# NVlabs/long-video-gan

Measured on NVIDIA H100. Metric: frames/sec (G+D train step: every convolution and torch_utils.ops call of the forward/backward passes, replayed), higher is better.
Workload: dtype f32

## Files before the change

### long-video-gan_b200/csrc/conv_igemm.cu

```cuda

#include <algorithm>
#include <cuda.h>
#include <stdlib.h>

#include "common.cuh"
#include "wgmma.cuh"
#include "conv_engine.cuh"

namespace lvg {
bool pw_supported(int dtype, int groups, int cin, int cout, int kt, int kh, int kw, int pad_t, int pad_h, int pad_w, int stride, int64_t P);
int pw_conv(const float* x, const float* w, float* y, int n, int cin, int cout, int64_t P, int64_t w_sco, int64_t w_sci, cudaStream_t s);
bool pw_tc_supported(int dtype, int groups, int cin, int cout, int kt, int kh, int kw, int pad_t, int pad_h, int pad_w, int stride, int64_t P);
int pw_tc_conv(const void* x, const void* w, void* y, int dtype, int n, int ck, int cm, int64_t P, int64_t w_sm, int64_t w_sk, void* workspace,
               int64_t workspace_bytes, cudaStream_t s, const void* res = nullptr, float rscale = 1.f);
int64_t pw_tc_workspace(int dtype, int ck, int cm);
}

namespace lvg {
namespace {

using namespace tc;

constexpr int kBM = 128;
constexpr int kATile = kBM * 16 * 2;
// ... 679 lines not shown
        set_error("convnd_fprop: outside the tensor-core kernel's envelope");
        return LVG_UNSUPPORTED;
    }
    IgemmJob j = fprop_job(sh, x, w, y);
    j.bias = bias; j.act = act; j.alpha = alpha; j.gain = gain; j.clamp = clamp;
    return run_igemm(j, workspace, workspace_bytes, (cudaStream_t)stream);
}

extern "C" int lvg_convnd_dgrad(const void* dy, const void* w, void* dx, int dtype, int n, int groups, int cin, int cout, int t, int h, int wd,
                                int kt, int kh, int kw, int pad_t, int pad_h, int pad_w, int stride, void* workspace, int64_t workspace_bytes,
                                void* stream)
{
    LVG_REQUIRE(dy && w && dx, "convnd_dgrad: dy, w, dx must not be NULL");
    const int route = lvg_convnd_route(1, dtype, n, groups, cin, cout, t, h, wd, kt, kh, kw, pad_t, pad_h, pad_w, stride, 0);
    if (route == 1) return pw_conv((const float*)dy, (const float*)w, (float*)dx, n, cout, cin, (int64_t)t * h * wd, 1, cin, (cudaStream_t)stream);
    if (route == 2 && aligned16(dy) && aligned16(dx))
        return pw_tc_conv(dy, w, dx, dtype, n, cout, cin, (int64_t)t * h * wd, 1, cin, workspace, workspace_bytes, (cudaStream_t)stream);
    const ConvShape sh = {dtype, n, groups, cin, cout, t, h, wd, kt, kh, kw, pad_t, pad_h, pad_w, stride};
    if (!sh.dgrad_ok()) {
        set_error("convnd_dgrad: outside the tensor-core kernel's envelope");
        return LVG_UNSUPPORTED;
    }
    return run_igemm(dgrad_job(sh, dy, w, dx), workspace, workspace_bytes, (cudaStream_t)stream);
}



namespace lvg {
namespace {

struct WgradV2Params {
    void* dw;
    int out_f32;
    int bf16, split;
    int n, groups, cin, cout;
    int to, ho;
    int kt, kh, kw, pad_t, pad_h, pad_w;
    int nt;
    int nblk_a, nblk_b;
    int lo_a, lo_b;
    int nseg, seg_w[4], seg_x0[4], ps[4];
    int rh;
    int khc;
    int ablk;
    int nsplit;
    int a_bytes, b_bytes, stage_bytes, stages;
    int64_t split_stride;
    int mrows;
    int tail_bytes;
};

struct WgradMaps { CUtensorMap a[4]; CUtensorMap b; };

template <bool BF16, int TAPS, int NT>
__global__ void __launch_bounds__(kIgemmThreads, 1) conv_wgrad_v2_kernel(const __grid_constant__ WgradMaps maps, const WgradV2Params p)
{
    extern __shared__ __align__(128) unsigned char smem_raw[];
    __shared__ uint64_t full_bar[kMaxStages], empty_bar[kMaxStages];
    unsigned char* smem = reinterpret_cast<unsigned char*>((reinterpret_cast<uintptr_t>(smem_raw) + 127) & ~(uintptr_t)127);

    const int warp = threadIdx.x / 32, lane = threadIdx.x % 32;
    const int wg = __shfl_sync(0xffffffffu, (int)threadIdx.x / 128, 0);
    int bx = blockIdx.x;
    const int sp = bx % p.nsplit; bx /= p.nsplit;
    int ky0 = 0;
    if (p.khc == 1) { ky0 = bx % p.kh; bx /= p.kh; }
    const int kt = bx % p.kt;
    const int nti = bx / p.kt;
    const int mti = blockIdx.y, g = blockIdx.z;
    const int nop = p.split ? 2 : 1;
    const int consumers = p.mrows / 64;

    const int rblocks = (p.ho + p.rh - 1) / p.rh;
    const int per_plane = p.nseg * rblocks;
    const int total = p.n * p.to * per_plane;
    const int s0 = (int)((int64_t)total * sp / p.nsplit), s1 = (int)((int64_t)total * (sp + 1) / p.nsplit);

    if (threadIdx.x == 0) {
        for (int s = 0; s < p.stages; s++) { mbar_init(&full_bar[s], 1); mbar_init(&empty_bar[s], (uint32_t)consumers); }
        fence_barrier_init();
    }
    for (int i = threadIdx.x; i < (p.stages * p.stage_bytes + p.tail_bytes) / 16; i += kIgemmThreads) reinterpret_cast<uint4*>(smem)[i] = make_uint4(0u, 0u, 0u, 0u);
    fence_proxy_async();
    __syncthreads();

    if (wg == 0) {
        if (warp == 0 && elect_one()) {
            for (int s = s0; s < s1; s++) {
                const int it = s - s0, slot = it % p.stages;
                if (it >= p.stages) mbar_wait(&empty_bar[slot], (uint32_t)((it / p.stages - 1) & 1));
                int r = s;
                const int rb = r % rblocks; r /= rblocks;
                const int seg = r % p.nseg; r /= p.nseg;
                const int t = r % p.to;
                const int n = r / p.to;
                const int inst = n * p.groups + g;
                unsigned char* st = smem + (size_t)slot * p.stage_bytes;
                mbar_expect_tx(&full_bar[slot], (uint32_t)(nop * (p.a_bytes + p.b_bytes)));
                const int oy0 = rb * p.rh;
                for (int o = 0; o < nop; o++) {
                    tma_load_4d(st + (size_t)o * p.a_bytes, &maps.a[seg], 0, oy0, t, inst * p.nblk_a + o * p.lo_a + mti * 16, &full_bar[slot]);
                    tma_load_4d(st + (size_t)nop * p.a_bytes + (size_t)o * p.b_bytes, &maps.b, 2 * (p.seg_x0[seg] - p.pad_w), oy0 + ky0 - p.pad_h,
                                t + kt - p.pad_t, inst * p.nblk_b + o * p.lo_b + nti * (NT / 8), &full_bar[slot]);
                }
            }
        }
    } else if (wg >= 1 && wg - 1 < consumers) {
        const int cw = wg - 1;
        const int tid = threadIdx.x % 128, wq = tid / 32;
        float acc[TAPS][NT / 2];
#pragma unroll
        for (int tap = 0; tap < TAPS; tap++)
#pragma unroll
            for (int i = 0; i < NT / 2; i++) acc[tap][i] = 0.f;
        int prev = -1;
        for (int s = s0; s < s1; s++) {
            const int it = s - s0, slot = it % p.stages;
            const int seg = (s / rblocks) % p.nseg;
            const int rb = s % rblocks;
            const int rows = min(p.rh, p.ho - rb * p.rh);
            const int ksteps = (rows * p.ps[seg] + 15) / 16;
            const uint32_t blk_a = (uint32_t)(p.rh * p.ps[seg] * 16);
            const uint32_t blk_b = (uint32_t)((p.rh + p.khc - 1) * p.ps[seg] * 16);
            const uint32_t ky16 = (uint32_t)p.ps[seg];
            mbar_wait(&full_bar[slot], (uint32_t)((it / p.stages) & 1));
            wgmma_fence();
            const uint32_t a0 = smem_u32(smem + (size_t)slot * p.stage_bytes) + (uint32_t)cw * 8u * blk_a;
            const uint32_t b0 = smem_u32(smem + (size_t)slot * p.stage_bytes) + (uint32_t)(nop * p.a_bytes);
            const uint32_t a_hi = desc_hi(blk_a), b_hi = desc_hi(blk_b);
            for (int term = 0; term < (p.split ? 3 : 1); term++) {
                const uint32_t a_lo0 = desc_lo(a0 + (term == 1 ? (uint32_t)p.a_bytes : 0u), 128);
                const uint32_t b_lo0 = desc_lo(b0 + (term == 2 ? (uint32_t)p.b_bytes : 0u), 128);
                for (int k = 0; k < ksteps; k++) {
#pragma unroll
                    for (int tap = 0; tap < TAPS; tap++) {
                        const int kyi = tap / p.kw, kx = tap - kyi * p.kw;
                        wgmma_m64nNk16<BF16, NT, 1, 1>(acc[tap], a_lo0 + 16u * k, a_hi, b_lo0 + 16u * k + (uint32_t)kyi * ky16 + (uint32_t)kx, b_hi);
                    }
                }
            }
            wgmma_commit();
            wgmma_wait<1>();
            mbar_arrive_if(&empty_bar[prev >= 0 ? prev : 0], prev >= 0 && tid == 0);
            prev = slot;
        }
        wgmma_wait<0>();

        const int taps = p.kt * p.kh * p.kw;
        const int ci0 = nti * NT;
#pragma unroll
        for (int tap = 0; tap < TAPS; tap++) {
            const int kyi = tap / p.kw, kx = tap - kyi * p.kw;
            const int tapg = (kt * p.kh + ky0 + kyi) * p.kw + kx;
#pragma unroll
            for (int i = 0; i < NT / 2; i++) {
                const int co = mti * kBM + cw * 64 + wq * 16 + lane / 4 + 8 * ((i / 2) % 2);
                const int cil = (i / 4) * 8 + 2 * (lane % 4) + i % 2;
                if (co >= p.cout || ci0 + cil >= p.cin) continue;
                const int64_t off = (((int64_t)g * p.cout + co) * p.cin + ci0 + cil) * taps + tapg;
                const float v = acc[tap][i];
                if (p.nsplit > 1) reinterpret_cast<float*>(p.dw)[(int64_t)sp * p.split_stride + off] = v;
                else if (p.out_f32) reinterpret_cast<float*>(p.dw)[off] = v;
                else reinterpret_cast<__half*>(p.dw)[off] = __float2half_rn(v);
            }
        }
    }
}

template <class TOut>
__global__ void __launch_bounds__(256) conv_wgrad_reduce_kernel(const float* __restrict__ part, TOut* __restrict__ out, int64_t n, int nsplit, int64_t stride)
{
    for (int64_t i = (int64_t)blockIdx.x * blockDim.x + threadIdx.x; i < n; i += (int64_t)gridDim.x * blockDim.x) {
        float s = 0.f;
        for (int k = 0; k < nsplit; k++) s += part[(int64_t)k * stride + i];
        if constexpr (sizeof(TOut) == 2) out[i] = __float2half_rn(s);
        else out[i] = s;
    }
}

inline int wgrad_cpad_a(int cout) { return (cout < kBM && env_flag("LVG_WGRAD_COMPACT", 1)) ? round_up(cout, 16) : round_up(cout, kBM); }

}

WgradPlan wgrad_plan(const ConvShape& s, bool fold)
{
    const int cin = s.cin, cout = s.cout, kh = s.kh, kw = s.kw;
    const int to = s.to(), ho = s.ho(), wo = s.wo();
    WgradPlan q;
    q.split = s.split();
    q.cpad_a = wgrad_cpad_a(cout);
    q.ablk = q.cpad_a < kBM ? q.cpad_a / 8 : 16;
    q.mrows = (q.cpad_a <= 64 && env_flag("LVG_WGRAD_M64", 1)) ? 64 : kBM;
    q.cpad_b = round_up(cin, 16);
    q.khc = (fold && kh > 1 && kh * kw * 32 <= 256 && cin <= env_flag("LVG_WGRAD_FOLD_CIN", 32) && env_flag("LVG_WGRAD_FOLD", 1)) ? kh : 1;
    int nt_cap = (256 / (q.khc * kw)) / 32 * 32;
// ... 12 lines not shown
        const int min_rows = q.ps % 16 != 0 ? 2 : 1;
        while (nt_cap > 32 && 2 * stage_of(min_rows, nt_cap) > 200 * 1024) nt_cap -= 32;
    }
    q.ntiles = (q.cpad_b + nt_cap - 1) / nt_cap;
    q.nt = round_up((q.cpad_b + q.ntiles - 1) / q.ntiles, 32);
    q.cpad_b = q.nt * q.ntiles;
    q.mt = (q.cpad_a + kBM - 1) / kBM;
    const int64_t inst = s.inst();
    q.a_bytes = inst * nop * (q.cpad_a / 8) * (int64_t)to * ho * wo * 16;
    q.b_bytes = inst * nop * (q.cpad_b / 8) * s.thw() * 16;
    q.dw_elems = (int64_t)s.groups * cout * cin * s.taps();
    q.rh = 1;
    while (q.rh < ho && q.rh < 255 - q.khc && stage_of(q.rh + 1, q.nt) <= 80 * 1024) q.rh++;
    if (q.ps % 16 != 0) q.rh = q.rh >= 2 ? q.rh / 2 * 2 : 2;
    for (;;) {
        q.a_stage = q.ablk * q.rh * q.ps * 16;
        q.b_stage = (q.nt / 8) * (q.rh + q.khc - 1) * q.ps * 16;
        q.stage_bytes = round_up(nop * (q.a_stage + q.b_stage), 128);
        const int over = (nop - 1) * q.a_stage + (q.mrows / 8) * q.rh * q.ps * 16 - q.stage_bytes;
        q.tail_bytes = round_up(256 + (over > 0 ? over : 0), 128);
        const int step = q.ps % 16 != 0 ? 2 : 1;
        if (2 * q.stage_bytes + q.tail_bytes <= 220 * 1024 || q.rh <= step) break;
        q.rh -= step;
    }
    q.stages = 2;
    while (q.stages < kMaxStages && (q.stages + 1) * q.stage_bytes + q.tail_bytes <= 220 * 1024) q.stages++;
    q.smem = (size_t)q.stages * q.stage_bytes + q.tail_bytes + 128;
    if (q.khc > 1 && q.smem > 227 * 1024) return wgrad_plan(s, false);
    const int64_t ctas = (int64_t)q.ntiles * (kh / q.khc) * s.kt * q.mt * s.groups;
    const int64_t stages = (int64_t)s.n * to * q.nseg * ((ho + q.rh - 1) / q.rh);
    const int sms = num_sms();
    int64_t cap = 160;
    if (cap > stages) cap = stages;
    while (cap > 1 && cap * q.dw_elems * 4 > (256ll << 20)) cap--;
    int64_t ns = 1;
    double best = 1e300;
    for (int64_t k = 1; k <= cap; k++) {
        const int64_t waves = (ctas * k + sms - 1) / sms;
        const double tm = (double)waves * ((double)((stages + k - 1) / k) + 4.0 * q.khc);
        if (tm < best * 0.999) { best = tm; ns = k; }
    }
    {
        const char* e = getenv("LVG_WGRAD_NSPLIT");
        if (e && atoi(e) >= 1) ns = atoi(e) < stages ? atoi(e) : stages;
    }
    q.nsplit = (int)ns;
    q.part_bytes = q.nsplit > 1 ? q.nsplit * q.dw_elems * 4 : 0;
    return q;
}

namespace {

typedef void (*WgradKernel)(const WgradMaps, const WgradV2Params);
template <bool B>
WgradKernel wgrad_kernel_of(int taps, int nt)
{
    switch (taps * 1000 + nt) {
    case 1032: return conv_wgrad_v2_kernel<B, 1, 32>;
    case 1064: return conv_wgrad_v2_kernel<B, 1, 64>;
    case 1096: return conv_wgrad_v2_kernel<B, 1, 96>;
    case 1128: return conv_wgrad_v2_kernel<B, 1, 128>;
    case 2032: return conv_wgrad_v2_kernel<B, 2, 32>;
    case 2064: return conv_wgrad_v2_kernel<B, 2, 64>;
    case 2096: return conv_wgrad_v2_kernel<B, 2, 96>;
    case 2128: return conv_wgrad_v2_kernel<B, 2, 128>;
    case 3032: return conv_wgrad_v2_kernel<B, 3, 32>;
    case 3064: return conv_wgrad_v2_kernel<B, 3, 64>;
    case 4032: return conv_wgrad_v2_kernel<B, 4, 32>;
    case 4064: return conv_wgrad_v2_kernel<B, 4, 64>;
    case 5032: return conv_wgrad_v2_kernel<B, 5, 32>;
    case 6032: return conv_wgrad_v2_kernel<B, 6, 32>;
    case 7032: return conv_wgrad_v2_kernel<B, 7, 32>;
    case 8032: return conv_wgrad_v2_kernel<B, 8, 32>;
    }
    if constexpr (!B) {
        switch (taps * 1000 + nt) {
        case 1160: return conv_wgrad_v2_kernel<B, 1, 160>;
        case 1192: return conv_wgrad_v2_kernel<B, 1, 192>;
        case 1224: return conv_wgrad_v2_kernel<B, 1, 224>;
        case 1256: return conv_wgrad_v2_kernel<B, 1, 256>;
        }
    }
    return nullptr;
}
WgradKernel wgrad_kernel(int split, int taps, int nt) { return split ? wgrad_kernel_of<true>(taps, nt) : wgrad_kernel_of<false>(taps, nt); }

bool dy8_tiles_agree(const ConvShape& s) { return wgrad_cpad_a(s.cout) == round_up(s.cout, 16); }

}

WgradRooms wgrad_rooms(const WgradPlan& q, bool dy8_pre) { return {dy8_pre ? 0 : round256(q.a_bytes), round256(q.b_bytes), q.part_bytes}; }

int run_wgrad(const ConvShape& sh, const void* x, const void* dy, void* dw, const WgradInputs& in, void* workspace, int64_t workspace_bytes,
              cudaStream_t s)
{
    const int to = sh.to(), ho = sh.ho(), wo = sh.wo();
    const WgradPlan q = wgrad_plan(sh);
    const WgradRooms r = wgrad_rooms(q, in.dy8_pre != nullptr);
    LVG_REQUIRE(workspace && workspace_bytes >= r.total(), "convnd_wgrad: workspace too small");
    LVG_REQUIRE(aligned16(workspace), "convnd_wgrad: workspace must be 16-byte aligned");
    LVG_REQUIRE(sh.groups <= 65535 && q.mt <= 65535, "convnd_wgrad: too many groups / channel tiles");
    const int64_t inst = sh.inst();
    unsigned char* ws = reinterpret_cast<unsigned char*>(workspace);
    unsigned char* dy8 = in.dy8_pre ? const_cast<unsigned char*>(in.dy8_pre) : ws;
    unsigned char* x8 = in.x8_pre ? const_cast<unsigned char*>(in.x8_pre) : ws + r.dy8;
    float* part = reinterpret_cast<float*>(ws + r.dy8 + r.x8);
    const int64_t thw_a = (int64_t)to * ho * wo, thw_b = sh.thw();
    {
        int rc = in.dy8_pre ? LVG_OK : pack_act(dy, dy8, q.split, inst, sh.cout, q.cpad_a / 8, to, sh.hos(), sh.wos(), ho, wo, sh.stride, s, in.dy_scale);
        if (rc) return rc;
        rc = in.x8_pre ? LVG_OK : pack_act(x, x8, q.split, inst, sh.cin, q.cpad_b / 8, sh.t, sh.h, sh.wd, sh.h, sh.wd, 1, s, in.x_scale);
        if (rc) return rc;
    }
    WgradV2Params p;
    memset(&p, 0, sizeof(p));
    p.out_f32 = q.split; p.bf16 = q.split; p.split = q.split;
    p.n = sh.n; p.groups = sh.groups; p.cin = sh.cin; p.cout = sh.cout; p.to = to; p.ho = ho;
    p.kt = sh.kt; p.kh = sh.kh; p.kw = sh.kw; p.pad_t = sh.pad_t; p.pad_h = sh.pad_h; p.pad_w = sh.pad_w;
    p.nt = q.nt;
    p.nblk_a = (q.split ? 2 : 1) * (q.cpad_a / 8); p.nblk_b = (q.split ? 2 : 1) * (q.cpad_b / 8);
    p.lo_a = q.cpad_a / 8; p.lo_b = q.cpad_b / 8;
    p.nseg = q.nseg;
    for (int j = 0; j < 4; j++) { p.seg_w[j] = q.seg_w[j]; p.seg_x0[j] = q.seg_x0[j]; p.ps[j] = q.ps; }
    p.rh = q.rh; p.khc = q.khc; p.ablk = q.ablk;
    p.mrows = q.mrows;
    p.a_bytes = q.a_stage; p.b_bytes = q.b_stage; p.stage_bytes = q.stage_bytes; p.stages = q.stages; p.tail_bytes = q.tail_bytes;
    const size_t smem = q.smem;
    LVG_REQUIRE(smem <= 227 * 1024, "convnd_wgrad: stage does not fit shared memory (%zu bytes)", smem);
    p.nsplit = q.nsplit;
    p.split_stride = q.dw_elems;
    p.dw = q.nsplit > 1 ? (void*)part : dw;
    WgradMaps maps;
    memset(&maps, 0, sizeof(maps));
    for (int j = 0; j < p.nseg; j++) {
        const int rc = encode_map(&maps.a[j], dy8 + (size_t)p.seg_x0[j] * 16, p.seg_w[j], ho, to, inst * p.nblk_a, wo, (int64_t)ho * wo, thw_a,
                                  p.ps[j], p.rh, 1, q.ablk);
        if (rc) return rc;
    }
    {
        const int rc = encode_map(&maps.b, x8, sh.wd, sh.h, sh.t, inst * p.nblk_b, sh.wd, (int64_t)sh.h * sh.wd, thw_b, p.ps[0], p.rh + q.khc - 1, 1,
                                  q.nt / 8);
        if (rc) return rc;
    }
    void (*const kern)(const WgradMaps, const WgradV2Params) = wgrad_kernel(q.split, q.khc * sh.kw, q.nt);
    LVG_REQUIRE(kern != nullptr, "convnd_wgrad: no kernel for %d taps x %d columns (split %d)", q.khc * sh.kw, q.nt, q.split);
    LVG_CUDA(cudaFuncSetAttribute(kern, cudaFuncAttributeMaxDynamicSharedMemorySize, (int)smem));
    dim3 grid((unsigned)(q.ntiles * sh.kt * (sh.kh / q.khc) * q.nsplit), (unsigned)q.mt, (unsigned)sh.groups);
    kern<<<grid, kIgemmThreads, smem, s>>>(maps, p);
    LVG_LAUNCH_CHECK();
    if (q.nsplit > 1) {
        int64_t blocks = (q.dw_elems + 255) / 256;
        const int64_t cap = (int64_t)num_sms() * 32;
        if (blocks > cap) blocks = cap;
        if (q.split) conv_wgrad_reduce_kernel<float><<<(unsigned)blocks, 256, 0, s>>>(part, (float*)dw, q.dw_elems, q.nsplit, q.dw_elems);
        else conv_wgrad_reduce_kernel<__half><<<(unsigned)blocks, 256, 0, s>>>(part, (__half*)dw, q.dw_elems, q.nsplit, q.dw_elems);
        LVG_LAUNCH_CHECK();
    }
    return LVG_OK;
}

bool shares_dy8(const ConvShape& s) { return env_flag("LVG_CONV_SHARED_DY8", 1) && dy8_tiles_agree(s); }

BackwardRooms backward_rooms(const ConvShape& s, bool shared)
{
    const Geometry gd = job_geometry(dgrad_job(s, nullptr, nullptr, nullptr));
    const WgradRooms wr = wgrad_rooms(wgrad_plan(s), shared);
    return {shared ? round256(gd.act_bytes) : 0, std::max(igemm_rooms_of(gd, shared).total(), wr.total()), wr.dy8};
}

int64_t backward_workspace(const ConvShape& s)
{
    const int64_t sep = backward_rooms(s, false).total();
    return dy8_tiles_agree(s) ? std::max(sep, backward_rooms(s, true).total()) : sep;
}

int backward_dgrad(const ConvShape& s, const void* dy, const float* d, const void* w, void* dx, void* workspace, int64_t workspace_bytes,
                   cudaStream_t st, Backward& b)
{
    const bool shared = shares_dy8(s);
    const BackwardRooms r = backward_rooms(s, shared);
    LVG_REQUIRE(workspace && aligned16(workspace) && workspace_bytes >= r.total(), "convnd backward: workspace too small or misaligned");
    unsigned char* ws = reinterpret_cast<unsigned char*>(workspace);
    b.dy8 = shared ? ws : nullptr;
    b.rest = ws + r.dy8;
    b.rest_bytes = workspace_bytes - r.dy8;
    b.x8 = b.rest + r.x8;
    IgemmJob j = dgrad_job(s, dy, w, dx);
    if (shared) {
        const int rc = pack_act(dy, ws, s.split(), s.inst(), s.cout, job_geometry(j).cblk, s.to(), s.hos(), s.wos(), s.ho(), s.wo(), s.stride, st, d);
        if (rc) return rc;
        j.x8_pre = ws;
    } else {
        j.in_scale = d;
    }
    return run_igemm(j, b.rest, b.rest_bytes, st);
}

int backward_wgrad(const ConvShape& s, const Backward& b, const void* x, const void* dy, const float* d, void* dw, const float* x_scale,
// ... 112 lines not shown
```

### long-video-gan_b200/csrc/wgmma.cuh

```cuda
#pragma once
#include "common.cuh"

namespace lvg {
namespace tc {

__device__ __forceinline__ uint32_t smem_u32(const void* p) { return (uint32_t)__cvta_generic_to_shared(p); }

__device__ __forceinline__ bool elect_one()
{
    uint32_t pred = 0;
    asm volatile(
        "{\n"
        " .reg .pred p;\n"
        " elect.sync _|p, 0xffffffff;\n"
        " selp.u32 %0, 1, 0, p;\n"
        "}\n"
        : "=r"(pred));
    return pred != 0;
}

__device__ __forceinline__ void mbar_init(uint64_t* bar, uint32_t count)
{
    asm volatile("mbarrier.init.shared::cta.b64 [%0], %1;" ::"r"(smem_u32(bar)), "r"(count));
}
// ... 25 lines not shown
__device__ __forceinline__ void bulk_copy_g2s(void* dst_smem, const void* src_gmem, uint32_t bytes, uint64_t* bar)
{
    asm volatile("cp.async.bulk.shared::cluster.global.mbarrier::complete_tx::bytes [%0], [%1], %2, [%3];" ::"r"(smem_u32(dst_smem)),
                 "l"(src_gmem), "r"(bytes), "r"(smem_u32(bar))
                 : "memory");
}
__device__ __forceinline__ void fence_barrier_init() { asm volatile("fence.mbarrier_init.release.cluster;" ::: "memory"); }
__device__ __forceinline__ void fence_proxy_async() { asm volatile("fence.proxy.async.shared::cta;" ::: "memory"); }

__device__ __forceinline__ uint32_t desc_lo(uint32_t saddr, uint32_t lbo_bytes) { return ((saddr >> 4) & 0x3fffu) | (((lbo_bytes >> 4) & 0x3fffu) << 16); }
__device__ __forceinline__ uint32_t desc_hi(uint32_t sbo_bytes) { return (sbo_bytes >> 4) & 0x3fffu; }

__device__ __forceinline__ void wgmma_fence() { asm volatile("wgmma.fence.sync.aligned;" ::: "memory"); }
__device__ __forceinline__ void wgmma_commit() { asm volatile("wgmma.commit_group.sync.aligned;" ::: "memory"); }
template <int N>
__device__ __forceinline__ void wgmma_wait() { asm volatile("wgmma.wait_group.sync.aligned %0;" ::"n"(N) : "memory"); }

#define LVG_D8(i)                                                                                                            \
    "+f"(d[i]), "+f"(d[i + 1]), "+f"(d[i + 2]), "+f"(d[i + 3]), "+f"(d[i + 4]), "+f"(d[i + 5]), "+f"(d[i + 6]), "+f"(d[i + 7])
#define LVG_WGMMA_ASM(NS, TYPE, REGS, A0, A1, B0, B1, TA_, TB_, SC)                                                           \
    "{\n .reg .b64 da, db;\n .reg .pred p;\n setp.ne.b32 p, %" SC ", 0;\n mov.b64 da, {%" A0 ", %" A1 "};\n"                   \
    " mov.b64 db, {%" B0 ", %" B1 "};\n wgmma.mma_async.sync.aligned.m64n" NS "k16.f32." TYPE "." TYPE " " REGS                 \
    ", da, db, p, 1, 1, %" TA_ ", %" TB_ ";\n}\n"
#define LVG_WGMMA(NS, REGS, A0, A1, B0, B1, TA_, TB_, SC, ...)                                                                \
    do {                                                                                                                       \
        if constexpr (BF16)                                                                                                    \
            asm volatile(LVG_WGMMA_ASM(NS, "bf16", REGS, A0, A1, B0, B1, TA_, TB_, SC)                                        \
                         : __VA_ARGS__ : "r"(a_lo), "r"(a_hi), "r"(b_lo), "r"(b_hi), "n"(TA), "n"(TB), "r"(1));               \
        else                                                                                                                   \
            asm volatile(LVG_WGMMA_ASM(NS, "f16", REGS, A0, A1, B0, B1, TA_, TB_, SC)                                         \
                         : __VA_ARGS__ : "r"(a_lo), "r"(a_hi), "r"(b_lo), "r"(b_hi), "n"(TA), "n"(TB), "r"(1));               \
    } while (0)
template <bool BF16, int N, int TA, int TB>
__device__ __forceinline__ void wgmma_m64nNk16(float (&d)[N / 2], uint32_t a_lo, uint32_t a_hi, uint32_t b_lo, uint32_t b_hi)
{
    static_assert(N % 16 == 0 && N >= 16 && N <= 256, "wgmma: N = 16, 32, ..., 256");
    if constexpr (N == 16) LVG_WGMMA("16", "{%0, %1, %2, %3, %4, %5, %6, %7}", "8", "9", "10", "11", "12", "13", "14", LVG_D8(0));
    else if constexpr (N == 32) LVG_WGMMA("32", "{%0, %1, %2, %3, %4, %5, %6, %7, %8, %9, %10, %11, %12, %13, %14, %15}", "16", "17", "18", "19", "20", "21", "22", LVG_D8(0), LVG_D8(8));
    else if constexpr (N == 48) LVG_WGMMA("48", "{%0, %1, %2, %3, %4, %5, %6, %7, %8, %9, %10, %11, %12, %13, %14, %15, %16, %17, %18, %19, %20, %21, %22, %23}", "24", "25", "26", "27", "28", "29", "30", LVG_D8(0), LVG_D8(8), LVG_D8(16));
    else if constexpr (N == 64) LVG_WGMMA("64", "{%0, %1, %2, %3, %4, %5, %6, %7, %8, %9, %10, %11, %12, %13, %14, %15, %16, %17, %18, %19, %20, %21, %22, %23, %24, %25, %26, %27, %28, %29, %30, %31}", "32", "33", "34", "35", "36", "37", "38", LVG_D8(0), LVG_D8(8), LVG_D8(16), LVG_D8(24));
    else if constexpr (N == 80) LVG_WGMMA("80", "{%0, %1, %2, %3, %4, %5, %6, %7, %8, %9, %10, %11, %12, %13, %14, %15, %16, %17, %18, %19, %20, %21, %22, %23, %24, %25, %26, %27, %28, %29, %30, %31, %32, %33, %34, %35, %36, %37, %38, %39}", "40", "41", "42", "43", "44", "45", "46", LVG_D8(0), LVG_D8(8), LVG_D8(16), LVG_D8(24), LVG_D8(32));
    else if constexpr (N == 96) LVG_WGMMA("96", "{%0, %1, %2, %3, %4, %5, %6, %7, %8, %9, %10, %11, %12, %13, %14, %15, %16, %17, %18, %19, %20, %21, %22, %23, %24, %25, %26, %27, %28, %29, %30, %31, %32, %33, %34, %35, %36, %37, %38, %39, %40, %41, %42, %43, %44, %45, %46, %47}", "48", "49", "50", "51", "52", "53", "54", LVG_D8(0), LVG_D8(8), LVG_D8(16), LVG_D8(24), LVG_D8(32), LVG_D8(40));
    else if constexpr (N == 112) LVG_WGMMA("112", "{%0, %1, %2, %3, %4, %5, %6, %7, %8, %9, %10, %11, %12, %13, %14, %15, %16, %17, %18, %19, %20, %21, %22, %23, %24, %25, %26, %27, %28, %29, %30, %31, %32, %33, %34, %35, %36, %37, %38, %39, %40, %41, %42, %43, %44, %45, %46, %47, %48, %49, %50, %51, %52, %53, %54, %55}", "56", "57", "58", "59", "60", "61", "62", LVG_D8(0), LVG_D8(8), LVG_D8(16), LVG_D8(24), LVG_D8(32), LVG_D8(40), LVG_D8(48));
    else if constexpr (N == 128) LVG_WGMMA("128", "{%0, %1, %2, %3, %4, %5, %6, %7, %8, %9, %10, %11, %12, %13, %14, %15, %16, %17, %18, %19, %20, %21, %22, %23, %24, %25, %26, %27, %28, %29, %30, %31, %32, %33, %34, %35, %36, %37, %38, %39, %40, %41, %42, %43, %44, %45, %46, %47, %48, %49, %50, %51, %52, %53, %54, %55, %56, %57, %58, %59, %60, %61, %62, %63}", "64", "65", "66", "67", "68", "69", "70", LVG_D8(0), LVG_D8(8), LVG_D8(16), LVG_D8(24), LVG_D8(32), LVG_D8(40), LVG_D8(48), LVG_D8(56));
    else if constexpr (N == 144) LVG_WGMMA("144", "{%0, %1, %2, %3, %4, %5, %6, %7, %8, %9, %10, %11, %12, %13, %14, %15, %16, %17, %18, %19, %20, %21, %22, %23, %24, %25, %26, %27, %28, %29, %30, %31, %32, %33, %34, %35, %36, %37, %38, %39, %40, %41, %42, %43, %44, %45, %46, %47, %48, %49, %50, %51, %52, %53, %54, %55, %56, %57, %58, %59, %60, %61, %62, %63, %64, %65, %66, %67, %68, %69, %70, %71}", "72", "73", "74", "75", "76", "77", "78", LVG_D8(0), LVG_D8(8), LVG_D8(16), LVG_D8(24), LVG_D8(32), LVG_D8(40), LVG_D8(48), LVG_D8(56), LVG_D8(64));
    else if constexpr (N == 160) LVG_WGMMA("160", "{%0, %1, %2, %3, %4, %5, %6, %7, %8, %9, %10, %11, %12, %13, %14, %15, %16, %17, %18, %19, %20, %21, %22, %23, %24, %25, %26, %27, %28, %29, %30, %31, %32, %33, %34, %35, %36, %37, %38, %39, %40, %41, %42, %43, %44, %45, %46, %47, %48, %49, %50, %51, %52, %53, %54, %55, %56, %57, %58, %59, %60, %61, %62, %63, %64, %65, %66, %67, %68, %69, %70, %71, %72, %73, %74, %75, %76, %77, %78, %79}", "80", "81", "82", "83", "84", "85", "86", LVG_D8(0), LVG_D8(8), LVG_D8(16), LVG_D8(24), LVG_D8(32), LVG_D8(40), LVG_D8(48), LVG_D8(56), LVG_D8(64), LVG_D8(72));
    else if constexpr (N == 176) LVG_WGMMA("176", "{%0, %1, %2, %3, %4, %5, %6, %7, %8, %9, %10, %11, %12, %13, %14, %15, %16, %17, %18, %19, %20, %21, %22, %23, %24, %25, %26, %27, %28, %29, %30, %31, %32, %33, %34, %35, %36, %37, %38, %39, %40, %41, %42, %43, %44, %45, %46, %47, %48, %49, %50, %51, %52, %53, %54, %55, %56, %57, %58, %59, %60, %61, %62, %63, %64, %65, %66, %67, %68, %69, %70, %71, %72, %73, %74, %75, %76, %77, %78, %79, %80, %81, %82, %83, %84, %85, %86, %87}", "88", "89", "90", "91", "92", "93", "94", LVG_D8(0), LVG_D8(8), LVG_D8(16), LVG_D8(24), LVG_D8(32), LVG_D8(40), LVG_D8(48), LVG_D8(56), LVG_D8(64), LVG_D8(72), LVG_D8(80));
    else if constexpr (N == 192) LVG_WGMMA("192", "{%0, %1, %2, %3, %4, %5, %6, %7, %8, %9, %10, %11, %12, %13, %14, %15, %16, %17, %18, %19, %20, %21, %22, %23, %24, %25, %26, %27, %28, %29, %30, %31, %32, %33, %34, %35, %36, %37, %38, %39, %40, %41, %42, %43, %44, %45, %46, %47, %48, %49, %50, %51, %52, %53, %54, %55, %56, %57, %58, %59, %60, %61, %62, %63, %64, %65, %66, %67, %68, %69, %70, %71, %72, %73, %74, %75, %76, %77, %78, %79, %80, %81, %82, %83, %84, %85, %86, %87, %88, %89, %90, %91, %92, %93, %94, %95}", "96", "97", "98", "99", "100", "101", "102", LVG_D8(0), LVG_D8(8), LVG_D8(16), LVG_D8(24), LVG_D8(32), LVG_D8(40), LVG_D8(48), LVG_D8(56), LVG_D8(64), LVG_D8(72), LVG_D8(80), LVG_D8(88));
    else if constexpr (N == 208) LVG_WGMMA("208", "{%0, %1, %2, %3, %4, %5, %6, %7, %8, %9, %10, %11, %12, %13, %14, %15, %16, %17, %18, %19, %20, %21, %22, %23, %24, %25, %26, %27, %28, %29, %30, %31, %32, %33, %34, %35, %36, %37, %38, %39, %40, %41, %42, %43, %44, %45, %46, %47, %48, %49, %50, %51, %52, %53, %54, %55, %56, %57, %58, %59, %60, %61, %62, %63, %64, %65, %66, %67, %68, %69, %70, %71, %72, %73, %74, %75, %76, %77, %78, %79, %80, %81, %82, %83, %84, %85, %86, %87, %88, %89, %90, %91, %92, %93, %94, %95, %96, %97, %98, %99, %100, %101, %102, %103}", "104", "105", "106", "107", "108", "109", "110", LVG_D8(0), LVG_D8(8), LVG_D8(16), LVG_D8(24), LVG_D8(32), LVG_D8(40), LVG_D8(48), LVG_D8(56), LVG_D8(64), LVG_D8(72), LVG_D8(80), LVG_D8(88), LVG_D8(96));
    else if constexpr (N == 224) LVG_WGMMA("224", "{%0, %1, %2, %3, %4, %5, %6, %7, %8, %9, %10, %11, %12, %13, %14, %15, %16, %17, %18, %19, %20, %21, %22, %23, %24, %25, %26, %27, %28, %29, %30, %31, %32, %33, %34, %35, %36, %37, %38, %39, %40, %41, %42, %43, %44, %45, %46, %47, %48, %49, %50, %51, %52, %53, %54, %55, %56, %57, %58, %59, %60, %61, %62, %63, %64, %65, %66, %67, %68, %69, %70, %71, %72, %73, %74, %75, %76, %77, %78, %79, %80, %81, %82, %83, %84, %85, %86, %87, %88, %89, %90, %91, %92, %93, %94, %95, %96, %97, %98, %99, %100, %101, %102, %103, %104, %105, %106, %107, %108, %109, %110, %111}", "112", "113", "114", "115", "116", "117", "118", LVG_D8(0), LVG_D8(8), LVG_D8(16), LVG_D8(24), LVG_D8(32), LVG_D8(40), LVG_D8(48), LVG_D8(56), LVG_D8(64), LVG_D8(72), LVG_D8(80), LVG_D8(88), LVG_D8(96), LVG_D8(104));
    else if constexpr (N == 240) LVG_WGMMA("240", "{%0, %1, %2, %3, %4, %5, %6, %7, %8, %9, %10, %11, %12, %13, %14, %15, %16, %17, %18, %19, %20, %21, %22, %23, %24, %25, %26, %27, %28, %29, %30, %31, %32, %33, %34, %35, %36, %37, %38, %39, %40, %41, %42, %43, %44, %45, %46, %47, %48, %49, %50, %51, %52, %53, %54, %55, %56, %57, %58, %59, %60, %61, %62, %63, %64, %65, %66, %67, %68, %69, %70, %71, %72, %73, %74, %75, %76, %77, %78, %79, %80, %81, %82, %83, %84, %85, %86, %87, %88, %89, %90, %91, %92, %93, %94, %95, %96, %97, %98, %99, %100, %101, %102, %103, %104, %105, %106, %107, %108, %109, %110, %111, %112, %113, %114, %115, %116, %117, %118, %119}", "120", "121", "122", "123", "124", "125", "126", LVG_D8(0), LVG_D8(8), LVG_D8(16), LVG_D8(24), LVG_D8(32), LVG_D8(40), LVG_D8(48), LVG_D8(56), LVG_D8(64), LVG_D8(72), LVG_D8(80), LVG_D8(88), LVG_D8(96), LVG_D8(104), LVG_D8(112));
    else if constexpr (N == 256) LVG_WGMMA("256", "{%0, %1, %2, %3, %4, %5, %6, %7, %8, %9, %10, %11, %12, %13, %14, %15, %16, %17, %18, %19, %20, %21, %22, %23, %24, %25, %26, %27, %28, %29, %30, %31, %32, %33, %34, %35, %36, %37, %38, %39, %40, %41, %42, %43, %44, %45, %46, %47, %48, %49, %50, %51, %52, %53, %54, %55, %56, %57, %58, %59, %60, %61, %62, %63, %64, %65, %66, %67, %68, %69, %70, %71, %72, %73, %74, %75, %76, %77, %78, %79, %80, %81, %82, %83, %84, %85, %86, %87, %88, %89, %90, %91, %92, %93, %94, %95, %96, %97, %98, %99, %100, %101, %102, %103, %104, %105, %106, %107, %108, %109, %110, %111, %112, %113, %114, %115, %116, %117, %118, %119, %120, %121, %122, %123, %124, %125, %126, %127}", "128", "129", "130", "131", "132", "133", "134", LVG_D8(0), LVG_D8(8), LVG_D8(16), LVG_D8(24), LVG_D8(32), LVG_D8(40), LVG_D8(48), LVG_D8(56), LVG_D8(64), LVG_D8(72), LVG_D8(80), LVG_D8(88), LVG_D8(96), LVG_D8(104), LVG_D8(112), LVG_D8(120));
}
#undef LVG_WGMMA
#undef LVG_WGMMA_ASM
#undef LVG_D8

}
}
```

Before: 2141.

## Load dy tile into registers via ldmatrix for multi-tap wgrad WGMMA

For weight-gradient kernels with two or more taps and 128-row tiles, the dy (A) operand is loaded once per k-step from shared memory into registers with ldmatrix.trans. It is then fed to the register-sourced WGMMA variant for every tap, instead of each tap re-reading A from shared memory through a descriptor. The k-steps are software-pipelined with triple-buffered fragments, committing per step with wait<2>. Per-tap B offsets are precomputed once. This adds register pressure, per-step commit/wait overhead, and a new asm path whose fragment layout must match the descriptor layout.

After: 2186, median of 6. +2.1%, better.

```diff
diff --git a/long-video-gan_b200/csrc/conv_igemm.cu b/long-video-gan_b200/csrc/conv_igemm.cu
--- a/long-video-gan_b200/csrc/conv_igemm.cu
+++ b/long-video-gan_b200/csrc/conv_igemm.cu
@@ -755,7 +755,7 @@
 
 struct WgradMaps { CUtensorMap a[4]; CUtensorMap b; };
 
-template <bool BF16, int TAPS, int NT>
+template <bool BF16, int TAPS, int NT, bool RA>
 __global__ void __launch_bounds__(kIgemmThreads, 1) conv_wgrad_v2_kernel(const __grid_constant__ WgradMaps maps, const WgradV2Params p)
 {
     extern __shared__ __align__(128) unsigned char smem_raw[];
@@ -816,6 +816,16 @@
         for (int tap = 0; tap < TAPS; tap++)
 #pragma unroll
             for (int i = 0; i < NT / 2; i++) acc[tap][i] = 0.f;
+        uint32_t tapoff[TAPS];
+        {
+            uint32_t row = 0;
+            int kx = 0;
+#pragma unroll
+            for (int tap = 0; tap < TAPS; tap++) {
+                tapoff[tap] = row + (uint32_t)kx;
+                if (++kx == p.kw) { kx = 0; row += (uint32_t)p.ps[0]; }
+            }
+        }
         int prev = -1;
         for (int s = s0; s < s1; s++) {
             const int it = s - s0, slot = it % p.stages;
@@ -825,25 +835,59 @@
             const int ksteps = (rows * p.ps[seg] + 15) / 16;
             const uint32_t blk_a = (uint32_t)(p.rh * p.ps[seg] * 16);
             const uint32_t blk_b = (uint32_t)((p.rh + p.khc - 1) * p.ps[seg] * 16);
-            const uint32_t ky16 = (uint32_t)p.ps[seg];
             mbar_wait(&full_bar[slot], (uint32_t)((it / p.stages) & 1));
-            wgmma_fence();
-            const uint32_t a0 = smem_u32(smem + (size_t)slot * p.stage_bytes) + (uint32_t)cw * 8u * blk_a;
             const uint32_t b0 = smem_u32(smem + (size_t)slot * p.stage_bytes) + (uint32_t)(nop * p.a_bytes);
-            const uint32_t a_hi = desc_hi(blk_a), b_hi = desc_hi(blk_b);
-            for (int term = 0; term < (p.split ? 3 : 1); term++) {
-                const uint32_t a_lo0 = desc_lo(a0 + (term == 1 ? (uint32_t)p.a_bytes : 0u), 128);
-                const uint32_t b_lo0 = desc_lo(b0 + (term == 2 ? (uint32_t)p.b_bytes : 0u), 128);
-                for (int k = 0; k < ksteps; k++) {
-#pragma unroll
-                    for (int tap = 0; tap < TAPS; tap++) {
-                        const int kyi = tap / p.kw, kx = tap - kyi * p.kw;
-                        wgmma_m64nNk16<BF16, NT, 1, 1>(acc[tap], a_lo0 + 16u * k, a_hi, b_lo0 + 16u * k + (uint32_t)kyi * ky16 + (uint32_t)kx, b_hi);
+            const uint32_t b_hi = desc_hi(blk_b);
+            if constexpr (RA) {
+                const uint32_t a0 = smem_u32(smem + (size_t)slot * p.stage_bytes) + (uint32_t)cw * 8u * blk_a +
+                                    (uint32_t)(2 * wq + (lane / 8) % 2) * blk_a + (uint32_t)(8 * (lane / 16) + lane % 8) * 16u;
+                const int nterms = p.split ? 3 : 1, nsteps = nterms * ksteps;
+                int k = 0, term = 0;
+                uint32_t a_cur = a0, b_cur = desc_lo(b0, 128);
+                auto kstep = [&](uint32_t (&f)[4]) {
+                    ldmatrix_x4_trans(f, a_cur);
+                    wgmma_fence();
+#pragma unroll
+                    for (int tap = 0; tap < TAPS; tap++) wgmma_m64nNk16_rs<BF16, NT, 1>(acc[tap], f, b_cur + tapoff[tap], b_hi);
+                    wgmma_commit();
+                    wgmma_wait<2>();
+                    if (++k < ksteps) {
+                        a_cur += 256u;
+                        b_cur += 16u;
+                    } else {
+                        k = 0;
+                        term++;
+                        a_cur = a0 + (term == 1 ? (uint32_t)p.a_bytes : 0u);
+                        b_cur = desc_lo(b0 + (term == 2 ? (uint32_t)p.b_bytes : 0u), 128);
+                    }
+                };
+                uint32_t fa[3][4];
+                for (int j = 0; j < nsteps; j += 3) {
+                    kstep(fa[0]);
+                    if (j + 1 < nsteps) {
+                        kstep(fa[1]);
+                        if (j + 2 < nsteps) kstep(fa[2]);
+                        else wgmma_wait<0>();
+                    } else {
+                        wgmma_wait<0>();
                     }
                 }
-            }
-            wgmma_commit();
-            wgmma_wait<1>();
+            } else {
+                wgmma_fence();
+                const uint32_t a_s = smem_u32(smem + (size_t)slot * p.stage_bytes) + (uint32_t)cw * 8u * blk_a;
+                const uint32_t a_hi = desc_hi(blk_a);
+                for (int term = 0; term < (p.split ? 3 : 1); term++) {
+                    const uint32_t a_lo0 = desc_lo(a_s + (term == 1 ? (uint32_t)p.a_bytes : 0u), 128);
+                    const uint32_t b_lo0 = desc_lo(b0 + (term == 2 ? (uint32_t)p.b_bytes : 0u), 128);
+                    for (int k = 0; k < ksteps; k++) {
+#pragma unroll
+                        for (int tap = 0; tap < TAPS; tap++)
+                            wgmma_m64nNk16<BF16, NT, 1, 1>(acc[tap], a_lo0 + 16u * k, a_hi, b_lo0 + 16u * k + tapoff[tap], b_hi);
+                    }
+                }
+                wgmma_commit();
+                wgmma_wait<1>();
+            }
             mbar_arrive_if(&empty_bar[prev >= 0 ? prev : 0], prev >= 0 && tid == 0);
             prev = slot;
         }
@@ -962,38 +1006,48 @@
 namespace {
 
 typedef void (*WgradKernel)(const WgradMaps, const WgradV2Params);
-template <bool B>
+template <bool B, bool RA>
 WgradKernel wgrad_kernel_of(int taps, int nt)
 {
+    if constexpr (!RA) {
+        switch (taps * 1000 + nt) {
+        case 1032: return conv_wgrad_v2_kernel<B, 1, 32, RA>;
+        case 1064: return conv_wgrad_v2_kernel<B, 1, 64, RA>;
+        case 1096: return conv_wgrad_v2_kernel<B, 1, 96, RA>;
+        case 1128: return conv_wgrad_v2_kernel<B, 1, 128, RA>;
+        }
+        if constexpr (!B) {
+            switch (taps * 1000 + nt) {
+            case 1160: return conv_wgrad_v2_kernel<B, 1, 160, RA>;
+            case 1192: return conv_wgrad_v2_kernel<B, 1, 192, RA>;
+            case 1224: return conv_wgrad_v2_kernel<B, 1, 224, RA>;
+            case 1256: return conv_wgrad_v2_kernel<B, 1, 256, RA>;
+            }
+        }
+    }
     switch (taps * 1000 + nt) {
-    case 1032: return conv_wgrad_v2_kernel<B, 1, 32>;
-    case 1064: return conv_wgrad_v2_kernel<B, 1, 64>;
-    case 1096: return conv_wgrad_v2_kernel<B, 1, 96>;
-    case 1128: return conv_wgrad_v2_kernel<B, 1, 128>;
-    case 2032: return conv_wgrad_v2_kernel<B, 2, 32>;
-    case 2064: return conv_wgrad_v2_kernel<B, 2, 64>;
-    case 2096: return conv_wgrad_v2_kernel<B, 2, 96>;
-    case 2128: return conv_wgrad_v2_kernel<B, 2, 128>;
-    case 3032: return conv_wgrad_v2_kernel<B, 3, 32>;
-    case 3064: return conv_wgrad_v2_kernel<B, 3, 64>;
-    case 4032: return conv_wgrad_v2_kernel<B, 4, 32>;
-    case 4064: return conv_wgrad_v2_kernel<B, 4, 64>;
-    case 5032: return conv_wgrad_v2_kernel<B, 5, 32>;
-    case 6032: return conv_wgrad_v2_kernel<B, 6, 32>;
-    case 7032: return conv_wgrad_v2_kernel<B, 7, 32>;
-    case 8032: return conv_wgrad_v2_kernel<B, 8, 32>;
-    }
-    if constexpr (!B) {
-        switch (taps * 1000 + nt) {
-        case 1160: return conv_wgrad_v2_kernel<B, 1, 160>;
-        case 1192: return conv_wgrad_v2_kernel<B, 1, 192>;
-        case 1224: return conv_wgrad_v2_kernel<B, 1, 224>;
-        case 1256: return conv_wgrad_v2_kernel<B, 1, 256>;
-        }
+    case 2032: return conv_wgrad_v2_kernel<B, 2, 32, RA>;
+    case 2064: return conv_wgrad_v2_kernel<B, 2, 64, RA>;
+    case 2096: return conv_wgrad_v2_kernel<B, 2, 96, RA>;
+    case 2128: return conv_wgrad_v2_kernel<B, 2, 128, RA>;
+    case 3032: return conv_wgrad_v2_kernel<B, 3, 32, RA>;
+    case 3064: return conv_wgrad_v2_kernel<B, 3, 64, RA>;
+    case 4032: return conv_wgrad_v2_kernel<B, 4, 32, RA>;
+    case 4064: return conv_wgrad_v2_kernel<B, 4, 64, RA>;
+    case 5032: return conv_wgrad_v2_kernel<B, 5, 32, RA>;
+    case 6032: return conv_wgrad_v2_kernel<B, 6, 32, RA>;
+    case 7032: return conv_wgrad_v2_kernel<B, 7, 32, RA>;
+    case 8032: return conv_wgrad_v2_kernel<B, 8, 32, RA>;
     }
     return nullptr;
 }
-WgradKernel wgrad_kernel(int split, int taps, int nt) { return split ? wgrad_kernel_of<true>(taps, nt) : wgrad_kernel_of<false>(taps, nt); }
+WgradKernel wgrad_kernel(int split, int taps, int nt, bool ra)
+{
+    if (ra) return split ? wgrad_kernel_of<true, true>(taps, nt) : wgrad_kernel_of<false, true>(taps, nt);
+    return split ? wgrad_kernel_of<true, false>(taps, nt) : wgrad_kernel_of<false, false>(taps, nt);
+}
+
+bool wgrad_dy_in_registers(const WgradPlan& q, int kw) { return q.khc * kw >= 2 && q.mrows == kBM; }
 
 bool dy8_tiles_agree(const ConvShape& s) { return wgrad_cpad_a(s.cout) == round_up(s.cout, 16); }
 
@@ -1052,8 +1106,10 @@
                                   q.nt / 8);
         if (rc) return rc;
     }
-    void (*const kern)(const WgradMaps, const WgradV2Params) = wgrad_kernel(q.split, q.khc * sh.kw, q.nt);
-    LVG_REQUIRE(kern != nullptr, "convnd_wgrad: no kernel for %d taps x %d columns (split %d)", q.khc * sh.kw, q.nt, q.split);
+    const bool ra = wgrad_dy_in_registers(q, sh.kw);
+    void (*const kern)(const WgradMaps, const WgradV2Params) = wgrad_kernel(q.split, q.khc * sh.kw, q.nt, ra);
+    LVG_REQUIRE(kern != nullptr, "convnd_wgrad: no kernel for %d taps x %d columns (split %d, dy in registers %d)", q.khc * sh.kw, q.nt,
+                q.split, (int)ra);
     LVG_CUDA(cudaFuncSetAttribute(kern, cudaFuncAttributeMaxDynamicSharedMemorySize, (int)smem));
     dim3 grid((unsigned)(q.ntiles * sh.kt * (sh.kh / q.khc) * q.nsplit), (unsigned)q.mt, (unsigned)sh.groups);
     kern<<<grid, kIgemmThreads, smem, s>>>(maps, p);
diff --git a/long-video-gan_b200/csrc/wgmma.cuh b/long-video-gan_b200/csrc/wgmma.cuh
--- a/long-video-gan_b200/csrc/wgmma.cuh
+++ b/long-video-gan_b200/csrc/wgmma.cuh
@@ -101,9 +101,53 @@
     else if constexpr (N == 240) LVG_WGMMA("240", "{%0, %1, %2, %3, %4, %5, %6, %7, %8, %9, %10, %11, %12, %13, %14, %15, %16, %17, %18, %19, %20, %21, %22, %23, %24, %25, %26, %27, %28, %29, %30, %31, %32, %33, %34, %35, %36, %37, %38, %39, %40, %41, %42, %43, %44, %45, %46, %47, %48, %49, %50, %51, %52, %53, %54, %55, %56, %57, %58, %59, %60, %61, %62, %63, %64, %65, %66, %67, %68, %69, %70, %71, %72, %73, %74, %75, %76, %77, %78, %79, %80, %81, %82, %83, %84, %85, %86, %87, %88, %89, %90, %91, %92, %93, %94, %95, %96, %97, %98, %99, %100, %101, %102, %103, %104, %105, %106, %107, %108, %109, %110, %111, %112, %113, %114, %115, %116, %117, %118, %119}", "120", "121", "122", "123", "124", "125", "126", LVG_D8(0), LVG_D8(8), LVG_D8(16), LVG_D8(24), LVG_D8(32), LVG_D8(40), LVG_D8(48), LVG_D8(56), LVG_D8(64), LVG_D8(72), LVG_D8(80), LVG_D8(88), LVG_D8(96), LVG_D8(104), LVG_D8(112));
     else if constexpr (N == 256) LVG_WGMMA("256", "{%0, %1, %2, %3, %4, %5, %6, %7, %8, %9, %10, %11, %12, %13, %14, %15, %16, %17, %18, %19, %20, %21, %22, %23, %24, %25, %26, %27, %28, %29, %30, %31, %32, %33, %34, %35, %36, %37, %38, %39, %40, %41, %42, %43, %44, %45, %46, %47, %48, %49, %50, %51, %52, %53, %54, %55, %56, %57, %58, %59, %60, %61, %62, %63, %64, %65, %66, %67, %68, %69, %70, %71, %72, %73, %74, %75, %76, %77, %78, %79, %80, %81, %82, %83, %84, %85, %86, %87, %88, %89, %90, %91, %92, %93, %94, %95, %96, %97, %98, %99, %100, %101, %102, %103, %104, %105, %106, %107, %108, %109, %110, %111, %112, %113, %114, %115, %116, %117, %118, %119, %120, %121, %122, %123, %124, %125, %126, %127}", "128", "129", "130", "131", "132", "133", "134", LVG_D8(0), LVG_D8(8), LVG_D8(16), LVG_D8(24), LVG_D8(32), LVG_D8(40), LVG_D8(48), LVG_D8(56), LVG_D8(64), LVG_D8(72), LVG_D8(80), LVG_D8(88), LVG_D8(96), LVG_D8(104), LVG_D8(112), LVG_D8(120));
 }
+
+#define LVG_WGMMA_RS_ASM(NS, TYPE, REGS, A0, A1, A2, A3, B0, B1, TB_, SC)                                                     \
+    "{\n .reg .b64 db;\n .reg .pred p;\n setp.ne.b32 p, %" SC ", 0;\n mov.b64 db, {%" B0 ", %" B1 "};\n"                       \
+    " wgmma.mma_async.sync.aligned.m64n" NS "k16.f32." TYPE "." TYPE " " REGS ", {%" A0 ", %" A1 ", %" A2 ", %" A3 "}, db, p, 1, 1, %" TB_ ";\n}\n"
+#define LVG_WGMMA_RS(NS, REGS, A0, A1, A2, A3, B0, B1, TB_, SC, ...)                                                          \
+    do {                                                                                                                       \
+        if constexpr (BF16)                                                                                                    \
+            asm volatile(LVG_WGMMA_RS_ASM(NS, "bf16", REGS, A0, A1, A2, A3, B0, B1, TB_, SC)                                  \
+                         : __VA_ARGS__ : "r"(a[0]), "r"(a[1]), "r"(a[2]), "r"(a[3]), "r"(b_lo), "r"(b_hi), "n"(TB), "r"(1));  \
+        else                                                                                                                   \
+            asm volatile(LVG_WGMMA_RS_ASM(NS, "f16", REGS, A0, A1, A2, A3, B0, B1, TB_, SC)                                   \
+                         : __VA_ARGS__ : "r"(a[0]), "r"(a[1]), "r"(a[2]), "r"(a[3]), "r"(b_lo), "r"(b_hi), "n"(TB), "r"(1));  \
+    } while (0)
+template <bool BF16, int N, int TB>
+__device__ __forceinline__ void wgmma_m64nNk16_rs(float (&d)[N / 2], const uint32_t (&a)[4], uint32_t b_lo, uint32_t b_hi)
+{
+    static_assert(N % 16 == 0 && N >= 16 && N <= 256, "wgmma: N = 16, 32, ..., 256");
+    if constexpr (N == 16) LVG_WGMMA_RS("16", "{%0, %1, %2, %3, %4, %5, %6, %7}", "8", "9", "10", "11", "12", "13", "14", "15", LVG_D8(0));
+    else if constexpr (N == 32) LVG_WGMMA_RS("32", "{%0, %1, %2, %3, %4, %5, %6, %7, %8, %9, %10, %11, %12, %13, %14, %15}", "16", "17", "18", "19", "20", "21", "22", "23", LVG_D8(0), LVG_D8(8));
+    else if constexpr (N == 48) LVG_WGMMA_RS("48", "{%0, %1, %2, %3, %4, %5, %6, %7, %8, %9, %10, %11, %12, %13, %14, %15, %16, %17, %18, %19, %20, %21, %22, %23}", "24", "25", "26", "27", "28", "29", "30", "31", LVG_D8(0), LVG_D8(8), LVG_D8(16));
+    else if constexpr (N == 64) LVG_WGMMA_RS("64", "{%0, %1, %2, %3, %4, %5, %6, %7, %8, %9, %10, %11, %12, %13, %14, %15, %16, %17, %18, %19, %20, %21, %22, %23, %24, %25, %26, %27, %28, %29, %30, %31}", "32", "33", "34", "35", "36", "37", "38", "39", LVG_D8(0), LVG_D8(8), LVG_D8(16), LVG_D8(24));
+    else if constexpr (N == 80) LVG_WGMMA_RS("80", "{%0, %1, %2, %3, %4, %5, %6, %7, %8, %9, %10, %11, %12, %13, %14, %15, %16, %17, %18, %19, %20, %21, %22, %23, %24, %25, %26, %27, %28, %29, %30, %31, %32, %33, %34, %35, %36, %37, %38, %39}", "40", "41", "42", "43", "44", "45", "46", "47", LVG_D8(0), LVG_D8(8), LVG_D8(16), LVG_D8(24), LVG_D8(32));
+    else if constexpr (N == 96) LVG_WGMMA_RS("96", "{%0, %1, %2, %3, %4, %5, %6, %7, %8, %9, %10, %11, %12, %13, %14, %15, %16, %17, %18, %19, %20, %21, %22, %23, %24, %25, %26, %27, %28, %29, %30, %31, %32, %33, %34, %35, %36, %37, %38, %39, %40, %41, %42, %43, %44, %45, %46, %47}", "48", "49", "50", "51", "52", "53", "54", "55", LVG_D8(0), LVG_D8(8), LVG_D8(16), LVG_D8(24), LVG_D8(32), LVG_D8(40));
+    else if constexpr (N == 112) LVG_WGMMA_RS("112", "{%0, %1, %2, %3, %4, %5, %6, %7, %8, %9, %10, %11, %12, %13, %14, %15, %16, %17, %18, %19, %20, %21, %22, %23, %24, %25, %26, %27, %28, %29, %30, %31, %32, %33, %34, %35, %36, %37, %38, %39, %40, %41, %42, %43, %44, %45, %46, %47, %48, %49, %50, %51, %52, %53, %54, %55}", "56", "57", "58", "59", "60", "61", "62", "63", LVG_D8(0), LVG_D8(8), LVG_D8(16), LVG_D8(24), LVG_D8(32), LVG_D8(40), LVG_D8(48));
+    else if constexpr (N == 128) LVG_WGMMA_RS("128", "{%0, %1, %2, %3, %4, %5, %6, %7, %8, %9, %10, %11, %12, %13, %14, %15, %16, %17, %18, %19, %20, %21, %22, %23, %24, %25, %26, %27, %28, %29, %30, %31, %32, %33, %34, %35, %36, %37, %38, %39, %40, %41, %42, %43, %44, %45, %46, %47, %48, %49, %50, %51, %52, %53, %54, %55, %56, %57, %58, %59, %60, %61, %62, %63}", "64", "65", "66", "67", "68", "69", "70", "71", LVG_D8(0), LVG_D8(8), LVG_D8(16), LVG_D8(24), LVG_D8(32), LVG_D8(40), LVG_D8(48), LVG_D8(56));
+    else if constexpr (N == 144) LVG_WGMMA_RS("144", "{%0, %1, %2, %3, %4, %5, %6, %7, %8, %9, %10, %11, %12, %13, %14, %15, %16, %17, %18, %19, %20, %21, %22, %23, %24, %25, %26, %27, %28, %29, %30, %31, %32, %33, %34, %35, %36, %37, %38, %39, %40, %41, %42, %43, %44, %45, %46, %47, %48, %49, %50, %51, %52, %53, %54, %55, %56, %57, %58, %59, %60, %61, %62, %63, %64, %65, %66, %67, %68, %69, %70, %71}", "72", "73", "74", "75", "76", "77", "78", "79", LVG_D8(0), LVG_D8(8), LVG_D8(16), LVG_D8(24), LVG_D8(32), LVG_D8(40), LVG_D8(48), LVG_D8(56), LVG_D8(64));
+    else if constexpr (N == 160) LVG_WGMMA_RS("160", "{%0, %1, %2, %3, %4, %5, %6, %7, %8, %9, %10, %11, %12, %13, %14, %15, %16, %17, %18, %19, %20, %21, %22, %23, %24, %25, %26, %27, %28, %29, %30, %31, %32, %33, %34, %35, %36, %37, %38, %39, %40, %41, %42, %43, %44, %45, %46, %47, %48, %49, %50, %51, %52, %53, %54, %55, %56, %57, %58, %59, %60, %61, %62, %63, %64, %65, %66, %67, %68, %69, %70, %71, %72, %73, %74, %75, %76, %77, %78, %79}", "80", "81", "82", "83", "84", "85", "86", "87", LVG_D8(0), LVG_D8(8), LVG_D8(16), LVG_D8(24), LVG_D8(32), LVG_D8(40), LVG_D8(48), LVG_D8(56), LVG_D8(64), LVG_D8(72));
+    else if constexpr (N == 176) LVG_WGMMA_RS("176", "{%0, %1, %2, %3, %4, %5, %6, %7, %8, %9, %10, %11, %12, %13, %14, %15, %16, %17, %18, %19, %20, %21, %22, %23, %24, %25, %26, %27, %28, %29, %30, %31, %32, %33, %34, %35, %36, %37, %38, %39, %40, %41, %42, %43, %44, %45, %46, %47, %48, %49, %50, %51, %52, %53, %54, %55, %56, %57, %58, %59, %60, %61, %62, %63, %64, %65, %66, %67, %68, %69, %70, %71, %72, %73, %74, %75, %76, %77, %78, %79, %80, %81, %82, %83, %84, %85, %86, %87}", "88", "89", "90", "91", "92", "93", "94", "95", LVG_D8(0), LVG_D8(8), LVG_D8(16), LVG_D8(24), LVG_D8(32), LVG_D8(40), LVG_D8(48), LVG_D8(56), LVG_D8(64), LVG_D8(72), LVG_D8(80));
+    else if constexpr (N == 192) LVG_WGMMA_RS("192", "{%0, %1, %2, %3, %4, %5, %6, %7, %8, %9, %10, %11, %12, %13, %14, %15, %16, %17, %18, %19, %20, %21, %22, %23, %24, %25, %26, %27, %28, %29, %30, %31, %32, %33, %34, %35, %36, %37, %38, %39, %40, %41, %42, %43, %44, %45, %46, %47, %48, %49, %50, %51, %52, %53, %54, %55, %56, %57, %58, %59, %60, %61, %62, %63, %64, %65, %66, %67, %68, %69, %70, %71, %72, %73, %74, %75, %76, %77, %78, %79, %80, %81, %82, %83, %84, %85, %86, %87, %88, %89, %90, %91, %92, %93, %94, %95}", "96", "97", "98", "99", "100", "101", "102", "103", LVG_D8(0), LVG_D8(8), LVG_D8(16), LVG_D8(24), LVG_D8(32), LVG_D8(40), LVG_D8(48), LVG_D8(56), LVG_D8(64), LVG_D8(72), LVG_D8(80), LVG_D8(88));
+    else if constexpr (N == 208) LVG_WGMMA_RS("208", "{%0, %1, %2, %3, %4, %5, %6, %7, %8, %9, %10, %11, %12, %13, %14, %15, %16, %17, %18, %19, %20, %21, %22, %23, %24, %25, %26, %27, %28, %29, %30, %31, %32, %33, %34, %35, %36, %37, %38, %39, %40, %41, %42, %43, %44, %45, %46, %47, %48, %49, %50, %51, %52, %53, %54, %55, %56, %57, %58, %59, %60, %61, %62, %63, %64, %65, %66, %67, %68, %69, %70, %71, %72, %73, %74, %75, %76, %77, %78, %79, %80, %81, %82, %83, %84, %85, %86, %87, %88, %89, %90, %91, %92, %93, %94, %95, %96, %97, %98, %99, %100, %101, %102, %103}", "104", "105", "106", "107", "108", "109", "110", "111", LVG_D8(0), LVG_D8(8), LVG_D8(16), LVG_D8(24), LVG_D8(32), LVG_D8(40), LVG_D8(48), LVG_D8(56), LVG_D8(64), LVG_D8(72), LVG_D8(80), LVG_D8(88), LVG_D8(96));
+    else if constexpr (N == 224) LVG_WGMMA_RS("224", "{%0, %1, %2, %3, %4, %5, %6, %7, %8, %9, %10, %11, %12, %13, %14, %15, %16, %17, %18, %19, %20, %21, %22, %23, %24, %25, %26, %27, %28, %29, %30, %31, %32, %33, %34, %35, %36, %37, %38, %39, %40, %41, %42, %43, %44, %45, %46, %47, %48, %49, %50, %51, %52, %53, %54, %55, %56, %57, %58, %59, %60, %61, %62, %63, %64, %65, %66, %67, %68, %69, %70, %71, %72, %73, %74, %75, %76, %77, %78, %79, %80, %81, %82, %83, %84, %85, %86, %87, %88, %89, %90, %91, %92, %93, %94, %95, %96, %97, %98, %99, %100, %101, %102, %103, %104, %105, %106, %107, %108, %109, %110, %111}", "112", "113", "114", "115", "116", "117", "118", "119", LVG_D8(0), LVG_D8(8), LVG_D8(16), LVG_D8(24), LVG_D8(32), LVG_D8(40), LVG_D8(48), LVG_D8(56), LVG_D8(64), LVG_D8(72), LVG_D8(80), LVG_D8(88), LVG_D8(96), LVG_D8(104));
+    else if constexpr (N == 240) LVG_WGMMA_RS("240", "{%0, %1, %2, %3, %4, %5, %6, %7, %8, %9, %10, %11, %12, %13, %14, %15, %16, %17, %18, %19, %20, %21, %22, %23, %24, %25, %26, %27, %28, %29, %30, %31, %32, %33, %34, %35, %36, %37, %38, %39, %40, %41, %42, %43, %44, %45, %46, %47, %48, %49, %50, %51, %52, %53, %54, %55, %56, %57, %58, %59, %60, %61, %62, %63, %64, %65, %66, %67, %68, %69, %70, %71, %72, %73, %74, %75, %76, %77, %78, %79, %80, %81, %82, %83, %84, %85, %86, %87, %88, %89, %90, %91, %92, %93, %94, %95, %96, %97, %98, %99, %100, %101, %102, %103, %104, %105, %106, %107, %108, %109, %110, %111, %112, %113, %114, %115, %116, %117, %118, %119}", "120", "121", "122", "123", "124", "125", "126", "127", LVG_D8(0), LVG_D8(8), LVG_D8(16), LVG_D8(24), LVG_D8(32), LVG_D8(40), LVG_D8(48), LVG_D8(56), LVG_D8(64), LVG_D8(72), LVG_D8(80), LVG_D8(88), LVG_D8(96), LVG_D8(104), LVG_D8(112));
+    else if constexpr (N == 256) LVG_WGMMA_RS("256", "{%0, %1, %2, %3, %4, %5, %6, %7, %8, %9, %10, %11, %12, %13, %14, %15, %16, %17, %18, %19, %20, %21, %22, %23, %24, %25, %26, %27, %28, %29, %30, %31, %32, %33, %34, %35, %36, %37, %38, %39, %40, %41, %42, %43, %44, %45, %46, %47, %48, %49, %50, %51, %52, %53, %54, %55, %56, %57, %58, %59, %60, %61, %62, %63, %64, %65, %66, %67, %68, %69, %70, %71, %72, %73, %74, %75, %76, %77, %78, %79, %80, %81, %82, %83, %84, %85, %86, %87, %88, %89, %90, %91, %92, %93, %94, %95, %96, %97, %98, %99, %100, %101, %102, %103, %104, %105, %106, %107, %108, %109, %110, %111, %112, %113, %114, %115, %116, %117, %118, %119, %120, %121, %122, %123, %124, %125, %126, %127}", "128", "129", "130", "131", "132", "133", "134", "135", LVG_D8(0), LVG_D8(8), LVG_D8(16), LVG_D8(24), LVG_D8(32), LVG_D8(40), LVG_D8(48), LVG_D8(56), LVG_D8(64), LVG_D8(72), LVG_D8(80), LVG_D8(88), LVG_D8(96), LVG_D8(104), LVG_D8(112), LVG_D8(120));
+}
+#undef LVG_WGMMA_RS
+#undef LVG_WGMMA_RS_ASM
 #undef LVG_WGMMA
 #undef LVG_WGMMA_ASM
 #undef LVG_D8
 
+__device__ __forceinline__ void ldmatrix_x4_trans(uint32_t (&r)[4], uint32_t saddr)
+{
+    asm volatile("ldmatrix.sync.aligned.m8n8.x4.trans.shared.b16 {%0, %1, %2, %3}, [%4];"
+                 : "=r"(r[0]), "=r"(r[1]), "=r"(r[2]), "=r"(r[3])
+                 : "r"(saddr)
+                 : "memory");
+}
+
 }
 }
```
